# zz9tf/multimodal-fusion

Measured on AMD Instinct MI355X. Metric: similarity-pairs/sec (NxN cosine+top-k), higher is better.
Workload: dtype f16 MFMA scan + f32 exact re-rank; 1 GPU; N=262144 d=512 single-modality cosine + top-5, self excluded, f32 features, unit-norm Gaussian rows; rows_per_rank=262144, parallelism=single GPU, driver=single, scan_kernel=scan_b16x<f16> (v_mfma_f32_16x16x32_f16), col_splits=1, scan_grid=3088, fallback_rows=0, overflow_rows=0, query_order=False, near_duplicate_rows_estimate=0

## Files before the change

multimodal-fusion_amd/csrc/mmf_api.hip:

```cpp
#include <stdarg.h>
#include <string.h>

#include <algorithm>
#include <map>
#include <mutex>
#include <optional>
#include <utility>
#include <vector>

#include "mmf_host.h"

namespace mmf {

static thread_local char g_err[512] = "";

void set_error(const char* fmt, ...) {
  va_list ap;
  va_start(ap, fmt);
  vsnprintf(g_err, sizeof(g_err), fmt, ap);
  va_end(ap);
}

struct WsEntry { char* base = nullptr; size_t cap = 0; WsKept kept; };
static std::mutex g_ws_mu;
// ... 594 lines not shown
    const bool symmetric = sym_try && !fo.perm && fo.n_panels == 0;
    const CandLists L = view(symmetric);
    MMF_HIP(hipMemsetAsync(L.overflow, 0, (size_t)n * 4, s));
    MMF_TRY(flags.zero(s));
    EventTimer t_scan, t_sel, t_fb;
    EventTimer t_panel[16];
    int grid = 0;
    MMF_HIP(hipMemsetAsync(seed, 0x80, (size_t)n_seed * 4 * seed_stripes(), s));
    MMF_HIP(hipMemsetAsync(L.spill_cnt, 0, (size_t)n * 4, s));
    MMF_TRY(t_scan.start(profile, s));
    ScanB16Panel pn;
    pn.seed = seed; pn.seed_stride = n_seed;
    pn.share = (splits > 1 || fo.n_panels > 1) ? 1 : 0;
    ScanB16Problem sp(fo.q, fo.c, n, m, fo.m_pad_tiles, fo.dp, r.d, fo.f16, r.metric, kk);
    if (symmetric) {
      bool live, forward;
      symmetric_live_mode(&live, &forward);
      int phases; bool antipodal;
      symmetric_schedule_mode(&phases, &antipodal, sym_G);
      const WsKept tables{sym.sched, (n + 255) / 256, sym_G, forward ? 1 : 0, phases, antipodal ? 1 : 0};
      MMF_TRY(launch_scan_b16_sym(sp, SymLaunch{sym_G, live, forward, symmetric_prune_mode(), !(sym_kept == tables), phases, antipodal}, L,
                                  scan_scratch, sym, pn, s, &grid));
      if (sym_keep) *sym_keep = tables;
    } else if (fo.n_panels == 0) {
      if (wide) {
        CandLists Lw = L;
        if (!wide_sink_mode()) { Lw.spill_cnt = nullptr; Lw.spill_ids = nullptr; Lw.spill_cap = 0; Lw.spill_stacks = 0; }
        pn.sunk = seed + 2 * n_seed;
        MMF_TRY(launch_scan_b16w(sp, splits, Lw, pn, s, &grid));
      }
      else MMF_TRY(launch_scan_b16(sp, splits, L, scan_scratch, pn, s, &grid));
    } else {
      int list_base = 0;
      for (int p = 0; p < fo.n_panels; ++p) {
        const mmf_panel& P = fo.panels[p];
        if (P.ready_event) MMF_HIP(hipStreamWaitEvent(s, static_cast<hipEvent_t>(P.ready_event), 0));
        MMF_TRY(t_panel[p].start(profile, s));
        pn.list_base = list_base;
        list_base += 2 * panel_splits[p];
        pn.seg_len = (uint32_t)P.seg_len; pn.seg_stride = (uint32_t)P.seg_stride; pn.id_off = (uint32_t)P.id_base;
        sp.ZC = P.Z; sp.cb = P.cb; sp.m = P.m; sp.m_pad = P.m_pad;
        MMF_TRY(launch_scan_b16(sp, panel_splits[p], L, scan_scratch, pn, s, &grid));
        MMF_TRY(t_panel[p].stop(s));
      }
    }
    MMF_TRY(launch_scan_b16_audit(pn, L.overflow, n, s));
    if (const char* e = getenv("MMF_DEBUG_FLAG_ROWS")) {
      const int64_t f = atoll(e);
      if (f > 0) MMF_HIP(hipMemsetAsync(L.overflow, 1, (size_t)(f < n ? f : n) * 4, s));
    }
    MMF_TRY(t_scan.stop(s));
    if (symmetric && getenv("MMF_SYMMETRIC_DEBUG")) {
      MMF_HIP(hipStreamSynchronize(s));
      std::vector<uint32_t> hc((size_t)n), hl((size_t)sym_grid() * 8);
      uint32_t none = 0;
      MMF_HIP(hipMemcpy(hc.data(), sym_cnt, hc.size() * 4, hipMemcpyDeviceToHost));
      MMF_HIP(hipMemcpy(hl.data(), sym.log_cnt, hl.size() * 4, hipMemcpyDeviceToHost));
      MMF_HIP(hipMemcpy(&none, sym.none_cnt, 4, hipMemcpyDeviceToHost));
      unsigned long long tot = 0, logged = 0; uint32_t mx = 0, lmx = 0;
      for (uint32_t v : hc) { tot += v; if (v > mx) mx = v; }
      for (uint32_t v : hl) { logged += v; if (v > lmx) lmx = v; }
      bool live, forward;
      symmetric_live_mode(&live, &forward);
      int phases; bool antipodal;
      symmetric_schedule_mode(&phases, &antipodal, sym_G);
      const size_t first_b = (size_t)sym_schedule_phase_b_begin((n + 255) / 256, sym_G) * 8;
      unsigned long long logged_b = 0;
      for (size_t i = first_b; i < hl.size(); ++i) logged_b += hl[i];
      fprintf(stderr, "[mmf symmetric] G %d grid %lld %s %s: rows without a threshold %u, received entries %llu (%.1f per row, largest %u of %d), fullest wave log %u of %d, logged entries %llu (%.1f per row, filing %s), phases %d antipodal %d, logged by phase B %llu (%.1f per row)\n",
              sym_G, (long long)sym_grid(), live ? "live" : "frozen", forward ? "ahead" : "back", none, tot, (double)tot / (double)n, mx,
              kSymCap, lmx, kSymLogPerWave, logged, (double)logged / (double)n, symmetric_prune_mode() ? "pruned" : "complete",
              forward ? 1 : phases, (antipodal && !forward) ? 1 : 0, logged_b, (double)logged_b / (double)n);
    }
    if (select_wait_event) MMF_HIP(hipStreamWaitEvent(s, static_cast<hipEvent_t>(select_wait_event), 0));

    SelectProblem q = r.select();
    q.rx = fo.rx; q.cy = fo.cy; q.perm = fo.perm;
    q.fail_rows = flags.fail_rows; q.fail_count = flags.fail_count; q.cand_total = r.stats ? flags.cand_total : nullptr;
    q.two_pass = true;
    q.order_scratch = getenv("MMF_SELECT_UNORDERED") ? nullptr : order_scratch;
    q.out_stride = out_stride;
    if (leave_floors) { q.floor_key_out = floor_key_out; q.floor_id_out = floor_id_out; }
    MMF_TRY(t_sel.start(profile, s));
    MMF_TRY(launch_select(q, L, s));
    MMF_TRY(t_sel.stop(s));

    MMF_TRY(flags.read(r.stats != nullptr, s));
    const uint32_t* h_fail4 = flags.h_fail4;
    const uint32_t h_fail = h_fail4[0];
    failed_rows = h_fail;
    if (h_fail > 0 && getenv("MMF_DEBUG_PRINT_FLAGGED")) {
      const uint32_t nshow = h_fail < 8 ? h_fail : 8;
      int32_t rows[8];
      MMF_HIP(hipMemcpy(rows, flags.fail_rows, nshow * sizeof(int32_t), hipMemcpyDeviceToHost));
      for (uint32_t i = 0; i < nshow; ++i) {
        int32_t enc[2] = {0, 0};
        MMF_HIP(hipMemcpy(&enc[0], seed + rows[i], 4, hipMemcpyDeviceToHost));
        MMF_HIP(hipMemcpy(&enc[1], seed + n_seed + rows[i], 4, hipMemcpyDeviceToHost));
        auto dec = [](int32_t o) { int32_t b = o >= 0 ? o : (o ^ 0x7fffffff); float f; memcpy(&f, &b, 4); return f; };
        fprintf(stderr, "[mmf flagged] row %d: best threshold %.9g (enc %d)  best dropped key %.9g (enc %d)  overflow %u short %u\n",
                rows[i], dec(enc[0]), enc[0], dec(enc[1]), enc[1], h_fail4[1], h_fail4[2]);
      }
    }

    MMF_TRY(t_fb.start(profile && h_fail > 0, s));
    if (h_fail > 0 && (int64_t)h_fail <= kRowsExactMax && !leave_floors) {
      for (int64_t off = 0; off < (int64_t)h_fail; off += rows_exact_cap) {
        SelectProblem fq = q;
        fq.perm = nullptr;
        fq.row_ids = flags.fail_rows + off;
        fq.n_rows = ((int64_t)h_fail - off < rows_exact_cap) ? ((int64_t)h_fail - off) : rows_exact_cap;
        MMF_TRY(launch_rows_exact(fq, row_keys, s));
      }
    } else if (h_fail > 0) {
      ExactPass ex(r, fo.rx, fo.cy);
      ex.row_ids = flags.fail_rows; ex.n_ids = h_fail; ex.forced_splits = fb_splits;
      ex.out_stride = out_stride;
      if (leave_floors) { ex.floors_out = true; ex.row_floor_key = floor_key_out; ex.row_floor_id = floor_id_out; }
      ex.add(ExactGroup{0, (int64_t)h_fail, true, 0, m, r.k});
      Workspace aux;
      MMF_TRY(r.call.workspace(ex.image_bytes(), &aux, 1));
      MMF_TRY(XL.zero(s));
      MMF_TRY(ex.run(aux, XL));
    }
// ... 3869 lines not shown
```

multimodal-fusion_amd/csrc/mmf_host.h:

```cpp
#pragma once
#include <hip/hip_runtime.h>
#include <functional>
#include <optional>
#include <stdint.h>
#include <stdio.h>

#include <string>
#include <vector>

#include "../../include/mmf_hg.h"
#include "../../include/mmf_hg_topk.h"
#include "../../include/mmf_hg_topk16.h"
#include "../../include/ext/mmf_hg_topk16_seg.h"
#include "../../include/ext/mmf_hg_topk_xy.h"
#include "../../include/ext/mmf_hg_seg_exact.h"
#include "../../include/ext/mmf_hg_topk_anyk.h"
#include "../../include/ext/mmf_hg_kmeans_ragged.h"
#include "../../include/ext/mmf_hg_cross_seg.h"
#include "../../include/ext/mmf_hg_cross_seg16.h"
#include "../../include/ext/mmf_hg_cross_segw.h"
#include "../../include/ext/mmf_hg_fast_anyk.h"
#include "../../include/ext/mmf_hg_wide_anyk.h"
#include "../../include/ext/mmf_hg_seg_anyk.h"
#include "../../include/ext/mmf_hg_cross_seg_anyk.h"
// ... 89 lines not shown
    guard.emplace(device);
    if (!guard->ok) { set_error("hipSetDevice(%d) failed", device); return MMF_E_HIP; }
    s = stream;
    return MMF_OK;
  }
  int begin(size_t bytes) {
    MMF_TRY(begin());
    return workspace(bytes, &ws);
  }
  int workspace(size_t bytes, Workspace* out, int slot = 0) const {
    if (!guard) { set_error("%s: workspace before begin() (internal invariant)", who); return MMF_E_INTERNAL; }
    return get_workspace_slot(device, stream, slot, bytes, out);
  }

 private:
  int device; hipStream_t stream;
  std::optional<DeviceGuard> guard;
};


constexpr int64_t kAnyRows = -1;
int check_offsets(const char* who, const char* name, const int64_t* ptr, int64_t n_seg, int64_t min_seg, int64_t min_rows, int64_t rows);

inline size_t dtype_size(int dt) { return dt == MMF_F32 ? 4 : 2; }


int launch_row_scalars(const void* X, int64_t n, int64_t d, int dtype, int metric, float* out,
                       uint32_t* max_n, hipStream_t s);

struct CandLists {
  uint32_t* cnt;
  uint32_t* ids;
  uint32_t* overflow;
  int lists;
  int cap;
  float* keys = nullptr;
  float* margin = nullptr;
  int slot_ulp = 16;
  uint32_t* spill_cnt = nullptr;
  uint32_t* spill_ids = nullptr;
  int spill_cap = 0;
  int spill_stacks = 0;
  uint32_t* sym_cnt = nullptr;
  uint2* sym_ent = nullptr;
  int sym_cap = 0;
};

constexpr int kSymListPairs = 3;
int64_t sym_schedule_grid(int64_t nb, int G);
int64_t sym_schedule_phase_b_begin(int64_t nb, int G);
void sym_schedule_table(int64_t nb, int G, int launch, int32_t* out, bool forward = false, int phases = 1, bool antipodal = false);
int sym_default_group(int64_t nb);
constexpr int kSymCap = 512;
constexpr int kSymLogPerWave = 4096;
struct SymBuffers {
  float* thr = nullptr;
  uint32_t* log = nullptr;
  uint32_t* log_cnt = nullptr;
  int32_t* sched = nullptr;
  uint32_t* none_cnt = nullptr;
  static size_t bytes(int64_t n_pad, int64_t grid) {
    return ws_bytes(n_pad, 4) + ws_bytes((size_t)grid * 8 * kSymLogPerWave * 4, 4) + ws_bytes((size_t)grid * 8, 4) +
           ws_bytes((size_t)grid * 16, 4) + ws_bytes(4, 4);
  }
  void carve(Workspace& ws, int64_t n_pad, int64_t grid) {
    thr = ws.take<float>(n_pad); log = ws.take<uint32_t>((size_t)grid * 8 * kSymLogPerWave * 4);
    log_cnt = ws.take<uint32_t>((size_t)grid * 8); sched = ws.take<int32_t>((size_t)grid * 16); none_cnt = ws.take<uint32_t>(4);
  }
};

struct ScanB16Panel {
  int list_base = 0;
  uint32_t seg_len = 0, seg_stride = 0, id_off = 0;
  int32_t* seed = nullptr;
  int64_t seed_stride = 0;
  int share = 0;
  int32_t* sunk = nullptr;
};

int64_t prep_f32_rows(int64_t n);
int64_t prep_f32_dim(int64_t d);
size_t prep_f32_bytes(int64_t n, int64_t d);
int launch_prep_f32(const void* X, int64_t n, int64_t d, int dtype, const int32_t* row_ids, float* out, hipStream_t s);

struct ScanProblem {
  const void* X; int64_t n;
  const void* Y; int64_t m;
  const float* Xp = nullptr;
  const float* Yp = nullptr;
  int64_t d;
  int dtype;
  int metric;
  float lambda;
  int kk;
  const float* rx;
  const float* cy;
  const int32_t* row_ids;
  int64_t n_rows;
  int col_splits;
  const float* floor_key = nullptr;
  const uint32_t* floor_id = nullptr;
  const float *Pq = nullptr, *Pc = nullptr, *pnq = nullptr, *pnc = nullptr;
  int dp = 0;
  float lambda_g = 0.0f;
};

int scan_f32_cap(int kk);
int launch_scan_f32(const ScanProblem& p, const CandLists& L, hipStream_t s, int* grid_out);

std::vector<int64_t> seg_exact_table(const int64_t* x_ptr, const int64_t* y_ptr, int64_t S, int k, int exclude_self, int col_splits,
                                     int* ranges_out, std::vector<char>* served_out);
std::vector<int64_t> cross_seg_table(const int64_t* x_ptr, const int64_t* y_ptr, int64_t S, int k, int col_splits, int* ranges_out);
std::vector<int32_t> cross_seg16_table(const int64_t* x_ptr, const int64_t* y_ptr, int64_t S, int qt, int dp, int cap, int cand_budget,
                                       int col_splits, int* lists_out);
std::vector<int32_t> cross_segw_table(const int64_t* x_ptr, const int64_t* y_ptr, int64_t S, int cap, int cand_budget, int col_splits,
                                      int* lists_out);
int launch_scan_f32_seg(const ScanProblem& p, const CandLists& L, const int64_t* sched, int64_t grid, hipStream_t s, bool cross = false);

struct SelectProblem {
  const void* X; int64_t n; const void* Y; int64_t m; int64_t d; int dtype; int metric; float lambda;
// ... 277 lines not shown
```

multimodal-fusion_amd/csrc/mmf_scan_bf16.hip:

```cpp
#include <stdlib.h>

#include <type_traits>

#include "mmf_dev.h"
#include "mmf_host.h"

namespace mmf {

constexpr int B_CT = 32;
#ifndef MMF_B_CAP
#define MMF_B_CAP 15
#endif
constexpr int B_CAP = MMF_B_CAP;
constexpr int B_CAP_BIG = 16;
constexpr int B_CAP_WIDE = 32;

typedef __bf16 bf16x8_t __attribute__((ext_vector_type(8)));
typedef _Float16 f16x8_t __attribute__((ext_vector_type(8)));
typedef uint32_t u32x4 __attribute__((ext_vector_type(4)));

struct PrepArgs {
  const void* X; int64_t n; int64_t d; int dtype; int metric;
  const float* scal;
  const uint32_t* max_n;
// ... 140 lines not shown
  int d;
  int debug;
  unsigned long long* dbg;
  uint32_t* lids;
  uint32_t* cand_cnt; uint32_t* cand_ids; uint32_t* overflow;
  float* cand_keys;
  float* margin_out;
  uint32_t* spill_cnt; uint32_t* spill_ids; int spill_cap;
  int spill_stacks;
  const int32_t* sched;
  float* sym_thr;
  int sym_live;
  uint32_t* sym_log;
  uint32_t* sym_log_cnt;
  int sym_log_cap;
  const uint32_t* xbounds;
  const float* ceil;
};

enum { SEG_QPOS = 0, SEG_ROW0 = 1, SEG_NQ = 2, SEG_T0 = 3, SEG_T1 = 4, SEG_IDOFF = 5, SEG_ENTRY = 8 };
enum { SYM_RB = 0, SYM_B1 = 1, SYM_N1 = 2, SYM_B2 = 3, SYM_N2 = 4, SYM_SLOT = 5, SYM_PHASE = 6 };
enum { XSEG_SLOT = 5, XSEG_W0 = 6, XSEG_W1 = 7 };

__device__ __forceinline__ int32_t seed_enc(float f) {
  const int32_t b = __float_as_int(f);
  return b >= 0 ? b : (b ^ 0x7fffffff);
}
constexpr int32_t kSeedNone = (int32_t)0x80808080;

__device__ __forceinline__ float scan_margin(int metric, int d, int dp, int cap, float zn, float rn, float un, const uint32_t* maxima) {
  const float ZB = __uint_as_float(maxima[0]), RB = __uint_as_float(maxima[1]);
  const float UB = __uint_as_float(maxima[2]), CB = __uint_as_float(maxima[3]);
  const float g_acc = (float)(dp + 8) * 5.9604645e-8f;
  const float g_chain = (float)(d + 2) * 5.9604645e-8f;
  const float slot_eps = (cap <= 16) ? 1.9073486e-6f : 3.8146973e-6f;
  const float e1 = rn * ZB + un * RB + (g_acc + slot_eps) * (zn * ZB + CB);
  float e2;
  if (metric == MMF_DOT) e2 = g_chain * un * UB;
  else if (metric == MMF_COSINE) e2 = (g_chain + 4.7683716e-7f) * un * UB * 1.01f;
  else e2 = g_chain * un * UB + 2.3841858e-7f * (un * un + UB * UB);
  return 2.0f * (e1 + e2) * 1.001f + 1e-30f;
}

__device__ __forceinline__ void glds4(const void* gptr, const void* lptr) {
  __builtin_amdgcn_global_load_lds((const __attribute__((address_space(1))) void*)(gptr), (__attribute__((address_space(3))) void*)(lptr), 4, 0, 0);
}

#ifndef MMF_SYM_ABLATE
#define MMF_SYM_ABLATE 0
#endif
#ifndef MMF_SYM_EARLY_THR
#define MMF_SYM_EARLY_THR 1
#endif
#ifndef MMF_SYM_ABLATE_Q
#define MMF_SYM_ABLATE_Q 0
#endif
#ifndef MMF_SYM_COUNT
#define MMF_SYM_COUNT 0
#endif
template <int KS, bool F16, bool DBG, int NW, int TPB, int CAP, bool SPLITK = false, bool SEG = false, int SYM = 0, bool XSEG = false,
          bool CEIL = false>
__global__ __launch_bounds__(64 * NW, (NW == 8) ? 2 : 1) void scan_b16x_kernel(ScanB16Args a) {
  static_assert(!CEIL || (SYM == 0 && !DBG), "per-row ceilings: the plain and the table-driven schedules (SEG, XSEG) only");
  static_assert(!SPLITK || (TPB == 1 && NW == 8 && (KS % 8) == 0), "split-k pairs");
  static_assert(SYM == 0 || (!SPLITK && !SEG && !DBG && TPB == 2), "symmetric schedule: the d = 512 kernel only");
  static_assert(!XSEG || (SEG && SYM == 0 && !DBG), "the cross-segment mask rides on the table-driven schedule");
  constexpr int NQW = SPLITK ? NW / 2 : NW;
  constexpr int NTL = 64 * NQW;
  constexpr int QT = 32 * NQW;
  constexpr int STAGES = 2 * TPB;
  constexpr int ROWB = KS * 32;
  constexpr int TILEB = B_CT * ROWB;
  constexpr int PIECES = TILEB / 1024;
  constexpr int PPW = (PIECES + NW - 1) / NW;
  static_assert(PIECES % NW == 0, "piece distribution");
  extern __shared__ __attribute__((aligned(1024))) char smem[];
  char* tiles = smem;
  float* cbs = reinterpret_cast<float*>(smem + STAGES * TILEB);
  float* lkeys = cbs + STAGES * 64;
  uint32_t* lids = a.lids + (size_t)blockIdx.x * (SlotList<CAP, NTL>::SLOTS * NTL);
  f32x4* xch = reinterpret_cast<f32x4*>(lkeys + CAP * NTL);
  volatile int* ack = reinterpret_cast<volatile int*>(xch + NQW * 4 * 64);

  const int tid = threadIdx.x;
  const int lane = tid & 63;
  const int wave = __builtin_amdgcn_readfirstlane(tid >> 6);
  const int khalf = SPLITK ? wave / NQW : 0;
  const int qw = SPLITK ? wave % NQW : wave;
  const bool owner = khalf == 0;
  const int half = lane >> 5;
  const int g = lane >> 4;
  const int c16 = lane & 15;
  const int ownb = g & 1;
  const int c = c16 + 16 * ownb;

  int64_t rb;
  int split;
  int64_t t_begin, t_end, row0 = 0;
  int nq = 0;
  uint32_t id_off = a.id_off;
  int sym_n1 = 0, sym_skip = 0;
  int xw0 = 0, xw1 = 0;
  if constexpr (SYM != 0) {
    const int32_t* e = a.sched + (size_t)blockIdx.x * SEG_ENTRY;
    if (e[SYM_RB] < 0) return;
    rb = e[SYM_RB]; split = SYM == 2 ? e[SYM_SLOT] : 0;
// ... 25 lines not shown
    if (t_begin > t_end) t_begin = t_end;
  }
  const int64_t q0 = rb * QT;
  const int64_t T = t_end - t_begin;

  const int64_t qop = q0 + 32 * qw + c;
  const int64_t qpos = SEG ? row0 + 32 * qw + c : qop;
  const bool qvalid = (SEG ? (32 * qw + c < nq) : (qpos < a.n_rows)) && owner;

  float margin;
  {
    const float ZB = __uint_as_float(a.maxima[0]), RB = __uint_as_float(a.maxima[1]);
    const float UB = __uint_as_float(a.maxima[2]), CB = __uint_as_float(a.maxima[3]);
    const float zn = a.q_zn[qop], rn = a.q_rn[qop], un = a.q_un[qop];
    const float g_acc = (float)(KS * 16 + 8) * 5.9604645e-8f;
    const float g_chain = (float)(a.d + 2) * 5.9604645e-8f;
    const float slot_eps = (CAP <= 16) ? 1.9073486e-6f : 3.8146973e-6f;
    const float e1 = rn * ZB + un * RB + (g_acc + slot_eps) * (zn * ZB + CB);
    float e2;
    if (a.metric == MMF_DOT) e2 = g_chain * un * UB;
    else if (a.metric == MMF_COSINE) e2 = (g_chain + 4.7683716e-7f) * un * UB * 1.01f;
    else e2 = g_chain * un * UB + 2.3841858e-7f * (un * un + UB * UB);
    margin = 2.0f * (e1 + e2) * 1.001f + 1e-30f;
  }

  SlotList<CAP, NTL> list;
  list.init(lkeys + (tid & (NTL - 1)), lids + (tid & (NTL - 1)));
  if (!qvalid) list.thr = __builtin_huge_valf();
  else if (a.spill_cnt) {
    list.sink.cnt = a.spill_cnt; list.sink.ids = a.spill_ids; list.sink.cap = (uint32_t)a.spill_cap; list.sink.row = qpos;
    list.sink.seg_len = a.seg_len; list.sink.seg_stride = a.seg_stride; list.sink.id_off = id_off;
    if (DBG) list.sink.ablate = (a.debug & 128) ? 1 : 0;
    if (a.spill_stacks) list.sink.stacks = 1 + half;
  }
  float pub = -kFltMax;
  auto sync_seed = [&]() {
    if (!qvalid) return;
    bool rose = false;
    if (list.thr > pub && list.thr > list.lost) {
      pub = list.thr;
      atomicMax(a.seed + qpos, seed_enc(pub));
      rose = true;
    }
    if (!a.share) return;
    const int32_t o = __hip_atomic_load(a.seed + qpos, __ATOMIC_RELAXED, __HIP_MEMORY_SCOPE_AGENT);
    if (o > kSeedNone) {
      const float t = __int_as_float(o >= 0 ? o : (o ^ 0x7fffffff));
      if (t > list.thr) { list.thr = t; pub = t; }
    }
    if constexpr (SYM == 2) {
      if (rose && a.sym_live) __hip_atomic_store(a.sym_thr + qpos, list.thr, __ATOMIC_RELAXED, __HIP_MEMORY_SCOPE_AGENT);
    }
  };
  if (a.share) sync_seed();
  const bool seeded = !__any(list.thr == -kFltMax);

  constexpr int KS2 = SPLITK ? KS / 4 : KS / 2;
  const int kbyte = khalf * KS2 * 64;
  u32x4 qf[KS2][2];
  {
    const char* qbase = reinterpret_cast<const char*>(a.ZQ) + (q0 + 32 * qw + c16) * (int64_t)ROWB + g * 16 + kbyte;
#pragma unroll
    for (int s = 0; s < KS2; ++s) {
      qf[s][0] = *reinterpret_cast<const u32x4*>(qbase + s * 64);
      qf[s][1] = *reinterpret_cast<const u32x4*>(qbase + 16 * (int64_t)ROWB + s * 64);
    }
#pragma unroll
    for (int s = 0; s < KS2; ++s) { asm volatile("" : "+v"(qf[s][0])); asm volatile("" : "+v"(qf[s][1])); }
  }

  int lo[4];
#pragma unroll
  for (int j = 0; j < 4; ++j) lo[j] = c16 * ROWB + ((((4 * j + g) ^ c16) & 15) << 4);

  uint32_t src_off[PPW];
#pragma unroll
  for (int i = 0; i < PPW; ++i) {
    const int p = wave + NW * i;
    const int off = p * 1024 + lane * 16;
    const int r = off / ROWB;
    const int chunk = (off % ROWB) >> 4;
    const int src_chunk = (chunk & ~15) | ((chunk ^ r) & 15);
    src_off[i] = (uint32_t)(r * ROWB + src_chunk * 16);
  }
  const char* zc0 = reinterpret_cast<const char*>(a.ZC) + (SYM != 0 ? 0 : t_begin * (int64_t)TILEB);
  const char* cb0 = reinterpret_cast<const char*>(a.cb + (SYM != 0 ? 0 : t_begin * B_CT));
  const char* zt0 = SYM != 0 ? zc0 + t_begin * (int64_t)TILEB : zc0;
  const char* ct0 = SYM != 0 ? cb0 + t_begin * B_CT * 4 : cb0;
  const __amdgpu_buffer_rsrc_t zrsrc = __builtin_amdgcn_make_buffer_rsrc(const_cast<char*>(zc0), 0, -1, 0x00020000);
  auto issue_piece = [&](const char* tsrc, int stage, int i) {
    if (DBG && (a.debug & 2)) return;
    if (DBG && (a.debug & 32)) tsrc = zc0;
    __builtin_amdgcn_raw_ptr_buffer_load_lds(zrsrc, (__attribute__((address_space(3))) void*)(tiles + stage * TILEB + (wave + NW * i) * 1024),
                                             16, (int)src_off[i], (int)(uint32_t)(tsrc - zc0), 0, 0);
  };
  const __amdgpu_buffer_rsrc_t brsrc = __builtin_amdgcn_make_buffer_rsrc(const_cast<char*>(cb0), 0, -1, 0x00020000);
  auto issue_bias = [&](const char* bsrc, int stage) {
    const uint32_t l = __builtin_amdgcn_mbcnt_hi(~0u, __builtin_amdgcn_mbcnt_lo(~0u, 0u));
    if (l < 32)
      __builtin_amdgcn_raw_ptr_buffer_load_lds(brsrc, (__attribute__((address_space(3))) void*)(cbs + stage * 64), 4, (int)(l * 4u),
                                               (int)(uint32_t)(bsrc - cb0), 0, 0);
  };
  auto sym_thr_stage = [&](int stage) -> float* { return lkeys + CAP * NTL + stage * 32; };
  auto issue_thr = [&](const char* bsrc, int stage) {
    const __amdgpu_buffer_rsrc_t trsrc = __builtin_amdgcn_make_buffer_rsrc(a.sym_thr, 0, -1, 0x00020000);
    const uint32_t l = __builtin_amdgcn_mbcnt_hi(~0u, __builtin_amdgcn_mbcnt_lo(~0u, 0u));
// ... 73 lines not shown
      __builtin_amdgcn_sched_group_barrier(0x008, 4, 0);
    }
    return acc;
  };
  auto max_qb = [&](const Acc& x, int qb) -> float {
    const f32x4& p = x.t[0][qb];
    const f32x4& q = x.t[1][qb];
    return fmaxf(fmaxf(fmaxf(p[0], p[1]), fmaxf(p[2], p[3])), fmaxf(fmaxf(q[0], q[1]), fmaxf(q[2], q[3])));
  };
  auto mask_padding = [&](Acc& x, int tt) {
    const int64_t r0 = (int64_t)id_base + (int64_t)tt * B_CT + ((tt >= sym_n1) ? (int64_t)sym_skip * B_CT : 0);
    if (__builtin_expect(r0 + B_CT > a.m, 0)) {
#pragma unroll
      for (int cb = 0; cb < 2; ++cb) {
#pragma unroll
        for (int jj = 0; jj < 4; ++jj) {
          if (r0 + 16 * cb + 4 * g + jj >= a.m) { x.t[cb][0][jj] = kNegInf; x.t[cb][1][jj] = kNegInf; }
        }
      }
    }
  };
  auto mask_excluded = [&](Acc& x, int tt) {
    if (__builtin_expect(tt >= xw0 && tt < xw1, 0)) {
      if (owner) {
        const uint32_t* bq = a.xbounds + 2 * (q0 + 32 * qw + c16);
        const uint2 b0 = *reinterpret_cast<const uint2*>(bq);
        const uint2 b1 = *reinterpret_cast<const uint2*>(bq + 32);
        const uint32_t j0 = id_base + (uint32_t)tt * B_CT + 4u * (uint32_t)g;
#pragma unroll
        for (int cb = 0; cb < 2; ++cb) {
#pragma unroll
          for (int jj = 0; jj < 4; ++jj) {
            const uint32_t j = j0 + 16u * cb + jj;
            if ((uint32_t)(j - b0.x) < b0.y) x.t[cb][0][jj] = kNegInf;
            if ((uint32_t)(j - b1.x) < b1.y) x.t[cb][1][jj] = kNegInf;
          }
        }
      }
    }
  };
  float thr_q0, thr_q1;
  auto refresh_thr = [&]() {
    const float mine = list.thr;
    const float theirs = __shfl_xor(mine, 16);
    thr_q0 = ownb ? theirs : mine;
    thr_q1 = ownb ? mine : theirs;
  };
  refresh_thr();

  constexpr bool SYMCNT = SYM != 0 && MMF_SYM_COUNT != 0;
  float ablate_keep = -kFltMax;
  auto filter = [&](const Acc& acc, int tt, float m0, float m1) {
    if (SYM != 0 && (MMF_SYM_ABLATE_Q & SYM) != 0 && (MMF_SYM_ABLATE_Q & 4) != 0) ablate_keep = fmaxf(ablate_keep, fmaxf(m0, m1));
    if (__builtin_expect(!(DBG && (a.debug & 1)) && !(SYM != 0 && (MMF_SYM_ABLATE_Q & SYM) != 0) && __any((m0 >= thr_q0) || (m1 >= thr_q1)), 0)) {
      uint32_t id0 = id_base + (uint32_t)tt * B_CT;
      if constexpr (SYM != 0) id0 += (tt >= sym_n1) ? (uint32_t)(sym_skip * B_CT) : 0u;
      f32x16 v;
#pragma unroll
      for (int cb = 0; cb < 2; ++cb) {
#pragma unroll
        for (int j = 0; j < 4; ++j) {
          const float mine = ownb ? acc.t[cb][1][j] : acc.t[cb][0][j];
          const float give = ownb ? acc.t[cb][0][j] : acc.t[cb][1][j];
          v[4 * cb + j] = mine;
          v[8 + 4 * cb + j] = __shfl_xor(give, 16);
        }
      }
      if constexpr (CEIL) {
        float ce;
        if constexpr (XSEG) {
          const int ln = (int)__builtin_amdgcn_mbcnt_hi(~0u, __builtin_amdgcn_mbcnt_lo(~0u, 0u));
          ce = (a.ceil + (q0 + 32 * qw))[(ln & 15) + (ln & 16)];
        } else ce = a.ceil[qop];
#pragma unroll
        for (int r = 0; r < 16; ++r) v[r] = (v[r] > ce) ? kNegInf : v[r];
      }
      const int g4 = 4 * g;
      auto rowof = [g4](int r) -> uint32_t { return (uint32_t)((g4 ^ ((r & 8) >> 1)) + (r & 3) + 16 * ((r >> 2) & 1)); };
      const bool cold = (!seeded && tt < 32) || __any(list.thr == -kFltMax);
      if ((DBG && (a.debug & 8)) || SYMCNT) {
        const bool willc = __any(list.cnt >= CAP - 1);
        int nh = 0;
#pragma unroll
        for (int r = 0; r < 16; ++r) nh += (v[r] >= list.thr) ? 1 : 0;
        const int lanes_hit = __popcll(__ballot(nh > 0));
#pragma unroll
        for (int o = 32; o > 0; o >>= 1) nh += __shfl_xor(nh, o);
        if (lane == 0) {
          atomicAdd(a.dbg + 0, 1ull);
          atomicAdd(a.dbg + 1, cold ? 1ull : 0ull);
          atomicAdd(a.dbg + 2, (unsigned long long)nh);
          atomicAdd(a.dbg + 3, (!cold && willc) ? 1ull : 0ull);
          atomicAdd(a.dbg + 4, (unsigned long long)lanes_hit);
        }
      }
      unsigned long long ts0 = 0;
      if (DBG && (a.debug & 16)) ts0 = __builtin_amdgcn_s_memtime();
      list.template offer_tile<!(DBG && SPLITK)>(v, id0, rowof, a.kk, margin);
      if (DBG && (a.debug & 16) && lane == 0) {
        const unsigned long long dt = __builtin_amdgcn_s_memtime() - ts0;
        atomicAdd(a.dbg + (cold ? 4 : 5), dt);
        atomicAdd(a.dbg + (cold ? 6 : 7), 1ull);
      }
      refresh_thr();
    }
    if (((DBG && (a.debug & 8)) || SYMCNT) && lane == 0) atomicAdd(a.dbg + 5, 1ull);
    if (__builtin_expect(a.share && (tt & 63) == 63, 0)) { sync_seed(); refresh_thr(); }
  };

  uint32_t sym_wcnt = 0;
  auto sym_offer = [&](const Acc& x, int tt, const float* th) {
    const f32x4 th0 = *reinterpret_cast<const f32x4*>(th + 4 * g);
    const f32x4 th1 = *reinterpret_cast<const f32x4*>(th + 16 + 4 * g);
    bool any = false;
#pragma unroll
    for (int j = 0; j < 4; ++j) {
      any |= fmaxf(x.t[0][0][j], x.t[0][1][j]) >= th0[j];
      any |= fmaxf(x.t[1][0][j], x.t[1][1][j]) >= th1[j];
    }
    if (__builtin_expect(__any(any) && (MMF_SYM_ABLATE != 1 || a.sym_log_cap < 0), 0)) {
      const uint32_t cj0 = id_base + (uint32_t)tt * B_CT + ((tt >= sym_n1) ? (uint32_t)(sym_skip * B_CT) : 0u) + 4u * (uint32_t)g;
      const uint32_t qi0 = (uint32_t)(q0 + 32 * qw + c16);
      const bool sym_qv0 = q0 + 32 * qw + c16 < a.n_rows, sym_qv1 = q0 + 32 * qw + c16 + 16 < a.n_rows;
      uint32_t* lg = a.sym_log + ((size_t)blockIdx.x * NW + wave) * (size_t)a.sym_log_cap * 4;
      uint32_t m = 0;
#pragma unroll
      for (int cb = 0; cb < 2; ++cb) {
#pragma unroll
        for (int j = 0; j < 4; ++j) {
          const float tj = cb ? th1[j] : th0[j];
          const bool cv = (int64_t)(cj0 + 16u * cb + j) < a.n_rows;
          m |= (x.t[cb][0][j] >= tj && sym_qv0 && cv) ? (1u << (8 * cb + 2 * j)) : 0u;
          m |= (x.t[cb][1][j] >= tj && sym_qv1 && cv) ? (2u << (8 * cb + 2 * j)) : 0u;
        }
      }
      unsigned long long busy = __ballot(m != 0u);
      while (busy) {
        if (m != 0u) {
          const uint32_t b = (uint32_t)__builtin_ctz(m);
          m &= m - 1u;
          const float v = select16(b, x.t[0][0][0], x.t[0][1][0], x.t[0][0][1], x.t[0][1][1], x.t[0][0][2], x.t[0][1][2], x.t[0][0][3], x.t[0][1][3],
                                   x.t[1][0][0], x.t[1][1][0], x.t[1][0][1], x.t[1][1][1], x.t[1][0][2], x.t[1][1][2], x.t[1][0][3], x.t[1][1][3]);
          const uint32_t cj = cj0 + 16u * (b >> 3) + ((b >> 1) & 3u);
          const uint32_t at = sym_wcnt + __builtin_amdgcn_mbcnt_hi((uint32_t)(busy >> 32), __builtin_amdgcn_mbcnt_lo((uint32_t)busy, 0u));
          if (at < (uint32_t)a.sym_log_cap) {
            u32x4 ent;
            ent[0] = cj; ent[1] = qi0 + 16u * (b & 1u); ent[2] = __float_as_uint(v); ent[3] = 0u;
            if (MMF_SYM_ABLATE != 3) *reinterpret_cast<u32x4*>(lg + (size_t)at * 4) = ent;
          } else {
            atomicMax(a.lost + cj, 0x7fffffff);
          }
        }
        sym_wcnt += (uint32_t)__popcll(busy);
        busy = __ballot(m != 0u);
      }
    }
  };

  unsigned long long tw = 0, tf = 0, tc = 0, tv = 0, t0s = 0, t1s = 0, t2s = 0, t3s = 0, tvs = 0;
  const bool stamps = DBG && (a.debug & 16) != 0;
  Acc acc_prev;
  float m0_prev = kNegInf, m1_prev = kNegInf;
#pragma unroll
  for (int cb = 0; cb < 2; ++cb) {
#pragma unroll
    for (int j = 0; j < 4; ++j) { acc_prev.t[cb][0][j] = kNegInf; acc_prev.t[cb][1][j] = kNegInf; }
// ... 478 lines not shown
    int64_t sb = (bb / per) * 8 + (bb % 8), rbi = sb * G + (bb % per) / 8;
    if (phase_b) {
      if (sb >= h) continue;
    } else if (bb / per >= stretches) {
      if (bb % 8 != (ns - 1) % 8) continue;
      sb = ns - 1; rbi = ns * G + (bb % per) / 8;
    } else if (sb >= ns) continue;
    if (rbi >= nb) continue;
    int64_t b1 = 0, n1 = 0, b2 = 0, n2 = 0;
    if (launch == 0) {
      b1 = first_tile(sb); n1 = end_tile(sb) - b1;
      if (ns >= 2 && (ns % 2) == 0 && !antipodal) { const int64_t o = (sb + ns / 2) % ns; b2 = first_tile(o); n2 = end_tile(o) - b2; }
    } else if (phase_b) {
      b1 = first_tile(sb + ns - h); n1 = tiles - b1;
    } else {
      const bool anti = antipodal && sb >= ns / 2;
      if (h == 0 && !anti) continue;
      if (h > 0) {
        int64_t lo = forward ? sb + 1 : sb - h, hi = lo + h - 1;
        if (phases == 2) { if (lo < 0) lo = 0; }
        else {
          if (lo >= ns) { lo -= ns; hi -= ns; }
          if (lo < 0) { lo += ns; hi += ns; }
        }
        if (hi < lo) continue;
        if (hi < ns) { b1 = first_tile(lo); n1 = end_tile(hi) - b1; }
        else { b1 = first_tile(lo); n1 = end_tile(ns - 1) - b1; b2 = 0; n2 = end_tile(hi - ns); }
      }
      if (anti) {
        const int64_t o = sb - ns / 2;
        if (n1 == 0) { b1 = first_tile(o); n1 = end_tile(o) - b1; }
        else { b2 = first_tile(o); n2 = end_tile(o) - b2; }
      }
    }
    if (n2 == 0) b2 = b1 + n1;
    e[SYM_RB] = (int32_t)rbi; e[SYM_B1] = (int32_t)b1; e[SYM_N1] = (int32_t)n1; e[SYM_B2] = (int32_t)b2; e[SYM_N2] = (int32_t)n2;
    e[SYM_SLOT] = phase_b ? 1 : 0;
    e[SYM_PHASE] = launch == 0 || phases != 2 ? 0 : (phase_b ? 2 : 1);
  }
}

__global__ void sym_thr_kernel(const int32_t* seed, float* thr, int64_t n, int64_t n_pad, uint32_t* none_cnt) {
  const int64_t i = (int64_t)blockIdx.x * blockDim.x + threadIdx.x;
  if (i >= n_pad) return;
  if (i >= n) { thr[i] = __builtin_huge_valf(); return; }
  const int32_t o = seed[i];
  if (o > kSeedNone) { thr[i] = __int_as_float(o >= 0 ? o : (o ^ 0x7fffffff)); return; }
  thr[i] = -kFltMax;
  atomicAdd(none_cnt, 1u);
}

__global__ __launch_bounds__(256) void sym_scatter_kernel(const uint32_t* log, const uint32_t* log_cnt, int log_cap, uint32_t* sym_cnt,
                                                          uint2* sym_ent, int cap, int32_t* lost,
                                                          const int32_t* seed, int slot_ulp) {
  const uint32_t c = log_cnt[blockIdx.x];
  const u32x4* lg = reinterpret_cast<const u32x4*>(log) + (size_t)blockIdx.x * log_cap;
  for (uint32_t e = threadIdx.x; e < c; e += 256) {
    const u32x4 v = lg[e];
    if (seed) {
      const int32_t sd = seed[v[0]], b = (int32_t)v[2];
      if (sd > kSeedNone && (b >= 0 ? b : (b ^ 0x7fffffff)) + slot_ulp < sd) continue;
    }
    const uint32_t slot = atomicAdd(sym_cnt + v[0], 1u);
    if (slot < (uint32_t)cap) {
      sym_ent[(size_t)v[0] * cap + slot] = make_uint2(v[1], v[2]);
    } else {
      atomicMax(lost + v[0], 0x7fffffff);
    }
  }
}

size_t scan_b16_sym_scratch_bytes(int64_t n_rows, int G) {
  const int64_t nb = (n_rows + 255) / 256;
  return (size_t)sym_schedule_grid(nb, G) * 16 * 512 * 4 + 256;
}

int launch_scan_b16_sym(const ScanB16Problem& p, const SymLaunch& y, const CandLists& L, void* scratch, const SymBuffers& sb,
                        const ScanB16Panel& pn, hipStream_t s, int* grid_out) {
  const int64_t n = p.n_rows, nb = (n + 255) / 256, n_pad = nb * 256, grid = sym_schedule_grid(nb, y.G);
  if (p.metric != MMF_DOT && p.metric != MMF_COSINE) {
    set_error("scan_b16_sym: metric %d has a per-candidate bias, which the symmetric kernels do not apply", p.metric);
    return MMF_E_INTERNAL;
  }
  if (L.lists != 2 * kSymListPairs || L.cap != B_CAP || !L.keys || !L.margin || !L.sym_cnt || !pn.seed) { set_error("scan_b16_sym: lists missing"); return MMF_E_INTERNAL; }
  if (n_pad * 1024 >= (int64_t(1) << 32)) { set_error("scan_b16_sym: operand image beyond the 32-bit tile offsets"); return MMF_E_INTERNAL; }
  if (y.tables) {
    std::vector<int32_t> tab((size_t)grid * 2 * SEG_ENTRY);
    sym_schedule_table(nb, y.G, 0, tab.data(), y.forward, y.phases, y.antipodal);
    sym_schedule_table(nb, y.G, 1, tab.data() + (size_t)grid * SEG_ENTRY, y.forward, y.phases, y.antipodal);
    MMF_TRY(upload_table(s, sb.sched, tab.data(), tab.size() * 4));
  }
  MMF_HIP(hipMemsetAsync(L.sym_cnt, 0, (size_t)n * 4, s));
  MMF_HIP(hipMemsetAsync(L.cnt, 0, (size_t)n * L.lists * 4, s));
  MMF_HIP(hipMemsetAsync(sb.log_cnt, 0, (size_t)grid * 8 * 4, s));
  MMF_HIP(hipMemsetAsync(sb.none_cnt, 0, 16, s));
  ScanB16Args a = scan_args(p, L, pn, scratch);
  a.ZQ = p.ZC;
  a.tiles_total = n_pad / B_CT; a.row_blocks = nb;
  a.spill_stacks = 0;
  a.sched = sb.sched;
  a.sym_thr = sb.thr; a.sym_live = y.live ? 1 : 0; a.sym_log = sb.log; a.sym_log_cnt = sb.log_cnt; a.sym_log_cap = kSymLogPerWave;
#if MMF_SYM_COUNT
  static unsigned long long* dbuf = nullptr;
  if (!dbuf) MMF_HIP(hipMalloc(&dbuf, 128));
  a.dbg = dbuf;
  auto report = [&](int launch) -> int {
    unsigned long long h[8];
    MMF_HIP(hipMemcpyAsync(h, dbuf, 64, hipMemcpyDeviceToHost, s));
    MMF_HIP(hipStreamSynchronize(s));
    fprintf(stderr, "[mmf sym count] launch %d: wave-tiles=%llu visits=%llu (cold %llu) hits=%llu entry-compactions=%llu lanes-with-hit=%llu\n",
            launch, h[5], h[0], h[1], h[2], h[3], h[4]);
    return MMF_OK;
  };
  MMF_HIP(hipMemsetAsync(dbuf, 0, 128, s));
#endif
  MMF_TRY((launch_b16_t<32, 8, 2, B_CAP, false, false, 1>(a, p.f16, grid, s)));
#if MMF_SYM_COUNT
  MMF_TRY(report(0));
  MMF_HIP(hipMemsetAsync(dbuf, 0, 128, s));
#endif
  hipLaunchKernelGGL(sym_thr_kernel, dim3((unsigned)((n_pad + 255) / 256)), dim3(256), 0, s, pn.seed, sb.thr, n, n_pad, sb.none_cnt);
  MMF_LAUNCH_CHECK();
  a.sched = sb.sched + (size_t)grid * SEG_ENTRY; a.list_base = 2; a.share = 1;
  MMF_TRY((launch_b16_t<32, 8, 2, B_CAP, false, false, 2>(a, p.f16, grid, s)));
#if MMF_SYM_COUNT
  MMF_TRY(report(1));
#endif
  hipLaunchKernelGGL(sym_scatter_kernel, dim3((unsigned)(grid * 8)), dim3(256), 0, s, sb.log, sb.log_cnt, kSymLogPerWave, L.sym_cnt,
                     L.sym_ent, L.sym_cap, pn.seed + pn.seed_stride, y.prune ? pn.seed : nullptr, L.slot_ulp);
  MMF_LAUNCH_CHECK();
  if (grid_out) *grid_out = (int)(2 * grid);
  return MMF_OK;
}

}
```

Measured before the change: 2074 billion pairs/s.

## Log whole candidate-tile records in symmetric scan and filter them in scatter

```diff
diff --git a/multimodal-fusion_amd/csrc/mmf_api.hip b/multimodal-fusion_amd/csrc/mmf_api.hip
--- a/multimodal-fusion_amd/csrc/mmf_api.hip
+++ b/multimodal-fusion_amd/csrc/mmf_api.hip
@@ -670,14 +670,16 @@
     MMF_TRY(t_scan.stop(s));
     if (symmetric && getenv("MMF_SYMMETRIC_DEBUG")) {
       MMF_HIP(hipStreamSynchronize(s));
-      std::vector<uint32_t> hc((size_t)n), hl((size_t)sym_grid() * 8);
+      std::vector<uint32_t> hc((size_t)n), hl((size_t)sym_grid() * 8), hr((size_t)sym_grid() * 8);
       uint32_t none = 0;
       MMF_HIP(hipMemcpy(hc.data(), sym_cnt, hc.size() * 4, hipMemcpyDeviceToHost));
-      MMF_HIP(hipMemcpy(hl.data(), sym.log_cnt, hl.size() * 4, hipMemcpyDeviceToHost));
+      MMF_HIP(hipMemcpy(hl.data(), sym.val_cnt, hl.size() * 4, hipMemcpyDeviceToHost));
+      MMF_HIP(hipMemcpy(hr.data(), sym.log_cnt, hr.size() * 4, hipMemcpyDeviceToHost));
       MMF_HIP(hipMemcpy(&none, sym.none_cnt, 4, hipMemcpyDeviceToHost));
-      unsigned long long tot = 0, logged = 0; uint32_t mx = 0, lmx = 0;
+      unsigned long long tot = 0, logged = 0, records = 0; uint32_t mx = 0, lmx = 0;
       for (uint32_t v : hc) { tot += v; if (v > mx) mx = v; }
-      for (uint32_t v : hl) { logged += v; if (v > lmx) lmx = v; }
+      for (uint32_t v : hl) logged += v;
+      for (uint32_t v : hr) { records += v; if (v > lmx) lmx = v; }
       bool live, forward;
       symmetric_live_mode(&live, &forward);
       int phases; bool antipodal;
@@ -685,9 +687,9 @@
       const size_t first_b = (size_t)sym_schedule_phase_b_begin((n + 255) / 256, sym_G) * 8;
       unsigned long long logged_b = 0;
       for (size_t i = first_b; i < hl.size(); ++i) logged_b += hl[i];
-      fprintf(stderr, "[mmf symmetric] G %d grid %lld %s %s: rows without a threshold %u, received entries %llu (%.1f per row, largest %u of %d), fullest wave log %u of %d, logged entries %llu (%.1f per row, filing %s), phases %d antipodal %d, logged by phase B %llu (%.1f per row)\n",
+      fprintf(stderr, "[mmf symmetric] G %d grid %lld %s %s: rows without a threshold %u, received entries %llu (%.1f per row, largest %u of %d), fullest wave log %u of %d, logged entries %llu (%.1f per row, filing %s), records %llu, phases %d antipodal %d, logged by phase B %llu (%.1f per row)\n",
               sym_G, (long long)sym_grid(), live ? "live" : "frozen", forward ? "ahead" : "back", none, tot, (double)tot / (double)n, mx,
-              kSymCap, lmx, kSymLogPerWave, logged, (double)logged / (double)n, symmetric_prune_mode() ? "pruned" : "complete",
+              kSymCap, lmx, scan_b16_sym_log_cap(), logged, (double)logged / (double)n, symmetric_prune_mode() ? "pruned" : "complete", records,
               forward ? 1 : phases, (antipodal && !forward) ? 1 : 0, logged_b, (double)logged_b / (double)n);
     }
     if (select_wait_event) MMF_HIP(hipStreamWaitEvent(s, static_cast<hipEvent_t>(select_wait_event), 0));
diff --git a/multimodal-fusion_amd/csrc/mmf_host.h b/multimodal-fusion_amd/csrc/mmf_host.h
--- a/multimodal-fusion_amd/csrc/mmf_host.h
+++ b/multimodal-fusion_amd/csrc/mmf_host.h
@@ -165,20 +165,22 @@
 void sym_schedule_table(int64_t nb, int G, int launch, int32_t* out, bool forward = false, int phases = 1, bool antipodal = false);
 int sym_default_group(int64_t nb);
 constexpr int kSymCap = 512;
-constexpr int kSymLogPerWave = 4096;
+constexpr int kSymLogPerWave = 2304;
+int scan_b16_sym_log_cap();
 struct SymBuffers {
   float* thr = nullptr;
   uint32_t* log = nullptr;
   uint32_t* log_cnt = nullptr;
+  uint32_t* val_cnt = nullptr;
   int32_t* sched = nullptr;
   uint32_t* none_cnt = nullptr;
   static size_t bytes(int64_t n_pad, int64_t grid) {
-    return ws_bytes(n_pad, 4) + ws_bytes((size_t)grid * 8 * kSymLogPerWave * 4, 4) + ws_bytes((size_t)grid * 8, 4) +
+    return ws_bytes(n_pad, 4) + ws_bytes((size_t)grid * 8 * kSymLogPerWave * 16, 4) + 2 * ws_bytes((size_t)grid * 8, 4) +
            ws_bytes((size_t)grid * 16, 4) + ws_bytes(4, 4);
   }
   void carve(Workspace& ws, int64_t n_pad, int64_t grid) {
-    thr = ws.take<float>(n_pad); log = ws.take<uint32_t>((size_t)grid * 8 * kSymLogPerWave * 4);
-    log_cnt = ws.take<uint32_t>((size_t)grid * 8); sched = ws.take<int32_t>((size_t)grid * 16); none_cnt = ws.take<uint32_t>(4);
+    thr = ws.take<float>(n_pad); log = ws.take<uint32_t>((size_t)grid * 8 * kSymLogPerWave * 16);
+    log_cnt = ws.take<uint32_t>((size_t)grid * 8); val_cnt = ws.take<uint32_t>((size_t)grid * 8); sched = ws.take<int32_t>((size_t)grid * 16); none_cnt = ws.take<uint32_t>(4);
   }
 };
 
diff --git a/multimodal-fusion_amd/csrc/mmf_scan_bf16.hip b/multimodal-fusion_amd/csrc/mmf_scan_bf16.hip
--- a/multimodal-fusion_amd/csrc/mmf_scan_bf16.hip
+++ b/multimodal-fusion_amd/csrc/mmf_scan_bf16.hip
@@ -216,6 +216,12 @@
 #ifndef MMF_SYM_EARLY_THR
 #define MMF_SYM_EARLY_THR 1
 #endif
+#ifndef MMF_SYM_RECORDS
+#define MMF_SYM_RECORDS 1
+#endif
+#ifndef MMF_SYM_SCALAR_ANY
+#define MMF_SYM_SCALAR_ANY 1
+#endif
 #ifndef MMF_SYM_ABLATE_Q
 #define MMF_SYM_ABLATE_Q 0
 #endif
@@ -347,6 +353,8 @@
       if (rose && a.sym_live) __hip_atomic_store(a.sym_thr + qpos, list.thr, __ATOMIC_RELAXED, __HIP_MEMORY_SCOPE_AGENT);
     }
   };
+  constexpr bool SCALAR_ANY = SYM != 0 && MMF_SYM_SCALAR_ANY != 0;
+  auto sym_hits = [&](unsigned long long b) -> bool { asm("" : "+s"(b)); return b != 0ull; };
   if (a.share) sync_seed();
   const bool seeded = !__any(list.thr == -kFltMax);
 
@@ -526,7 +534,9 @@
   float ablate_keep = -kFltMax;
   auto filter = [&](const Acc& acc, int tt, float m0, float m1) {
     if (SYM != 0 && (MMF_SYM_ABLATE_Q & SYM) != 0 && (MMF_SYM_ABLATE_Q & 4) != 0) ablate_keep = fmaxf(ablate_keep, fmaxf(m0, m1));
-    if (__builtin_expect(!(DBG && (a.debug & 1)) && !(SYM != 0 && (MMF_SYM_ABLATE_Q & SYM) != 0) && __any((m0 >= thr_q0) || (m1 >= thr_q1)), 0)) {
+    if (__builtin_expect(!(DBG && (a.debug & 1)) && !(SYM != 0 && (MMF_SYM_ABLATE_Q & SYM) != 0) &&
+                         (SCALAR_ANY ? sym_hits(__builtin_amdgcn_ballot_w64(m0 >= thr_q0) | __builtin_amdgcn_ballot_w64(m1 >= thr_q1))
+                                     : __any((m0 >= thr_q0) || (m1 >= thr_q1)) != 0), 0)) {
       uint32_t id0 = id_base + (uint32_t)tt * B_CT;
       if constexpr (SYM != 0) id0 += (tt >= sym_n1) ? (uint32_t)(sym_skip * B_CT) : 0u;
       f32x16 v;
@@ -586,6 +596,48 @@
   auto sym_offer = [&](const Acc& x, int tt, const float* th) {
     const f32x4 th0 = *reinterpret_cast<const f32x4*>(th + 4 * g);
     const f32x4 th1 = *reinterpret_cast<const f32x4*>(th + 16 + 4 * g);
+    if constexpr (MMF_SYM_RECORDS != 0) {
+      bool any0 = false, any1 = false;
+      unsigned long long hit0 = 0ull, hit1 = 0ull;
+#pragma unroll
+      for (int j = 0; j < 4; ++j) {
+        const bool p0 = fmaxf(x.t[0][0][j], x.t[0][1][j]) >= th0[j], p1 = fmaxf(x.t[1][0][j], x.t[1][1][j]) >= th1[j];
+        any0 |= p0; any1 |= p1;
+        if constexpr (SCALAR_ANY) { hit0 |= __builtin_amdgcn_ballot_w64(p0); hit1 |= __builtin_amdgcn_ballot_w64(p1); }
+      }
+      if (__builtin_expect((SCALAR_ANY ? sym_hits(hit0 | hit1) : __any(any0 || any1) != 0) && (MMF_SYM_ABLATE != 1 || a.sym_log_cap < 0), 0)) {
+        const uint32_t cj0 = id_base + (uint32_t)tt * B_CT + ((tt >= sym_n1) ? (uint32_t)(sym_skip * B_CT) : 0u) + 4u * (uint32_t)g;
+        const uint32_t qi0 = (uint32_t)(q0 + 32 * qw + c16);
+        u32x4* lg = reinterpret_cast<u32x4*>(a.sym_log) + ((size_t)blockIdx.x * NW + wave) * (size_t)a.sym_log_cap * 4;
+#pragma unroll
+        for (int cb = 0; cb < 2; ++cb) {
+          const bool hit = cb ? any1 : any0;
+          const unsigned long long b = SCALAR_ANY ? (cb ? hit1 : hit0) : __ballot(hit);
+          if (hit) {
+            const uint32_t at = sym_wcnt + __builtin_amdgcn_mbcnt_hi((uint32_t)(b >> 32), __builtin_amdgcn_mbcnt_lo((uint32_t)b, 0u));
+            if (at < (uint32_t)a.sym_log_cap) {
+              if (MMF_SYM_ABLATE != 3) {
+                u32x4 hd;
+                hd[0] = cj0 + 16u * cb; hd[1] = qi0; hd[2] = 0u; hd[3] = 0u;
+                u32x4* r = lg + (size_t)at * 4;
+                r[0] = hd;
+                r[1] = __builtin_bit_cast(u32x4, cb ? th1 : th0);
+                r[2] = __builtin_bit_cast(u32x4, x.t[cb][0]);
+                r[3] = __builtin_bit_cast(u32x4, x.t[cb][1]);
+              }
+            } else {
+#pragma unroll
+              for (int jj = 0; jj < 4; ++jj) {
+                const uint32_t cj = cj0 + 16u * cb + jj;
+                if ((int64_t)cj < a.n_rows) atomicMax(a.lost + cj, 0x7fffffff);
+              }
+            }
+          }
+          sym_wcnt += (uint32_t)__popcll(b);
+        }
+      }
+      return;
+    }
     bool any = false;
 #pragma unroll
     for (int j = 0; j < 4; ++j) {
@@ -1170,8 +1222,37 @@
 
 __global__ __launch_bounds__(256) void sym_scatter_kernel(const uint32_t* log, const uint32_t* log_cnt, int log_cap, uint32_t* sym_cnt,
                                                           uint2* sym_ent, int cap, int32_t* lost,
-                                                          const int32_t* seed, int slot_ulp) {
+                                                          const int32_t* seed, int slot_ulp, int64_t n_rows, uint32_t* val_cnt) {
   const uint32_t c = log_cnt[blockIdx.x];
+#if MMF_SYM_RECORDS
+  __shared__ uint32_t passed_all;
+  if (c == 0) { if (threadIdx.x == 0) val_cnt[blockIdx.x] = 0u; return; }
+  if (threadIdx.x == 0) passed_all = 0u;
+  __syncthreads();
+  const uint32_t* lg = log + (size_t)blockIdx.x * log_cap * 16;
+  uint32_t passed = 0;
+  for (uint32_t e = threadIdx.x; e < 8u * c; e += 256) {
+    const uint32_t* r = lg + (size_t)(e >> 3) * 16;
+    const uint32_t vi = e & 7u, j = vi & 3u;
+    const uint32_t cj = r[0] + j, qi = r[1] + 16u * (vi >> 2), kb = r[8 + vi];
+    if (!(__uint_as_float(kb) >= __uint_as_float(r[4 + j])) || (int64_t)qi >= n_rows || (int64_t)cj >= n_rows) continue;
+    ++passed;
+    if (seed) {
+      const int32_t sd = seed[cj], b = (int32_t)kb;
+      if (sd > kSeedNone && (b >= 0 ? b : (b ^ 0x7fffffff)) + slot_ulp < sd) continue;
+    }
+    const uint32_t slot = atomicAdd(sym_cnt + cj, 1u);
+    if (slot < (uint32_t)cap) {
+      sym_ent[(size_t)cj * cap + slot] = make_uint2(qi, kb);
+    } else {
+      atomicMax(lost + cj, 0x7fffffff);
+    }
+  }
+  if (passed) atomicAdd(&passed_all, passed);
+  __syncthreads();
+  if (threadIdx.x == 0) val_cnt[blockIdx.x] = passed_all;
+#else
+  if (threadIdx.x == 0) val_cnt[blockIdx.x] = c;
   const u32x4* lg = reinterpret_cast<const u32x4*>(log) + (size_t)blockIdx.x * log_cap;
   for (uint32_t e = threadIdx.x; e < c; e += 256) {
     const u32x4 v = lg[e];
@@ -1186,6 +1267,16 @@
       atomicMax(lost + v[0], 0x7fffffff);
     }
   }
+#endif
+}
+
+int scan_b16_sym_log_cap() {
+  int cap = kSymLogPerWave * (MMF_SYM_RECORDS ? 1 : 4);
+  if (const char* e = getenv("MMF_SYMMETRIC_LOG_CAP")) {
+    const int v = atoi(e);
+    if (v >= 1 && v < cap) cap = v;
+  }
+  return cap;
 }
 
 size_t scan_b16_sym_scratch_bytes(int64_t n_rows, int G) {
@@ -1196,6 +1287,7 @@
 int launch_scan_b16_sym(const ScanB16Problem& p, const SymLaunch& y, const CandLists& L, void* scratch, const SymBuffers& sb,
                         const ScanB16Panel& pn, hipStream_t s, int* grid_out) {
   const int64_t n = p.n_rows, nb = (n + 255) / 256, n_pad = nb * 256, grid = sym_schedule_grid(nb, y.G);
+  const int log_cap = scan_b16_sym_log_cap();
   if (p.metric != MMF_DOT && p.metric != MMF_COSINE) {
     set_error("scan_b16_sym: metric %d has a per-candidate bias, which the symmetric kernels do not apply", p.metric);
     return MMF_E_INTERNAL;
@@ -1217,7 +1309,7 @@
   a.tiles_total = n_pad / B_CT; a.row_blocks = nb;
   a.spill_stacks = 0;
   a.sched = sb.sched;
-  a.sym_thr = sb.thr; a.sym_live = y.live ? 1 : 0; a.sym_log = sb.log; a.sym_log_cnt = sb.log_cnt; a.sym_log_cap = kSymLogPerWave;
+  a.sym_thr = sb.thr; a.sym_live = y.live ? 1 : 0; a.sym_log = sb.log; a.sym_log_cnt = sb.log_cnt; a.sym_log_cap = log_cap;
 #if MMF_SYM_COUNT
   static unsigned long long* dbuf = nullptr;
   if (!dbuf) MMF_HIP(hipMalloc(&dbuf, 128));
@@ -1244,8 +1336,8 @@
 #if MMF_SYM_COUNT
   MMF_TRY(report(1));
 #endif
-  hipLaunchKernelGGL(sym_scatter_kernel, dim3((unsigned)(grid * 8)), dim3(256), 0, s, sb.log, sb.log_cnt, kSymLogPerWave, L.sym_cnt,
-                     L.sym_ent, L.sym_cap, pn.seed + pn.seed_stride, y.prune ? pn.seed : nullptr, L.slot_ulp);
+  hipLaunchKernelGGL(sym_scatter_kernel, dim3((unsigned)(grid * 8)), dim3(256), 0, s, sb.log, sb.log_cnt, log_cap, L.sym_cnt,
+                     L.sym_ent, L.sym_cap, pn.seed + pn.seed_stride, y.prune ? pn.seed : nullptr, L.slot_ulp, n, sb.val_cnt);
   MMF_LAUNCH_CHECK();
   if (grid_out) *grid_out = (int)(2 * grid);
   return MMF_OK;
```

Measured after the change: 2133 billion pairs/s (median of 6 runs). +2.9%, better.
